# sanje2v/DualSuperResLearningForSemSeg

Hardware: AMD Instinct MI355X
Metric: stage-3 train images/sec at 256x512->512x1024 (higher is better)
Workload: dtype f32; 1 GPU; DSRL stage 3 (ResNet-101 OS16 + ASPP + SSSR/SISR decoders + FA loss), full train step, random-init weights, 256x512 input -> 512x1024 logits; global_batch=8, per_gpu_batch=8, parallelism=dp1, optimizer=SGD m0.9 wd5e-4 lr0.006

## Files before the change

dualsuperreslearningforsemseg_amd/_lib.py:

```python
import ctypes as C
import os

import torch

_HERE = os.path.dirname(os.path.abspath(__file__))
LIB_PATH = os.path.join(_HERE, 'libdsrl_hip.so')

fp = C.c_void_p
i32 = C.c_int
i64 = C.c_int64
u64 = C.c_uint64
u32 = C.c_uint32
f32 = C.c_float
sz = C.c_size_t
stream_t = C.c_void_p

_conv_shape = [i32] * 10


class WgradProblem(C.Structure):
    _fields_ = [('x', C.c_void_p), ('dy', C.c_void_p), ('dw', C.c_void_p)] + [(n, C.c_int32) for n in
                ('ldx', 'lddy', 'N', 'H', 'W', 'C', 'K', 'R', 'S', 'stride', 'pad', 'dil')] + [('x_amax', C.c_void_p), ('dy_amax', C.c_void_p)]


PROTOTYPES = {
    'dsrl_version': (i32, []),
    'dsrl_last_error': (C.c_char_p, []),
    'dsrl_device_check': (i32, [C.POINTER(i32)]),
    'dsrl_conv2d_fwd_workspace_bytes': (sz, _conv_shape),
    'dsrl_conv2d_fwd': (i32, [fp, i32, fp, fp, fp, i32] + _conv_shape + [fp, sz, stream_t]),
    'dsrl_conv2d_fwd_stats_parts': (i32, _conv_shape),
    'dsrl_conv2d_fwd_stats': (i32, [fp, i32, fp, fp, fp, i32] + _conv_shape + [fp, sz, fp, i32, stream_t]),
    'dsrl_conv2d_dgrad_workspace_bytes': (sz, _conv_shape),
    'dsrl_conv2d_transposed_filter_floats': (sz, [i32] * 4),
    'dsrl_conv2d_transpose_filter': (i32, [fp, fp, i32, i32, i32, i32, stream_t]),
    'dsrl_conv2d_transpose_filters_batched': (i32, [fp, i32, i64, stream_t]),
    'dsrl_conv2d_filters_amax_segment_floats': (i32, []),
    'dsrl_conv2d_filters_amax_batched': (i32, [fp, i64, stream_t]),
    'dsrl_conv2d_dgrad': (i32, [fp, i32, fp, fp, fp, i32] + _conv_shape + [fp, sz, stream_t]),
    'dsrl_conv2d_dgrad_stats_parts': (i32, _conv_shape),
    'dsrl_conv2d_dgrad_bnstats': (i32, [fp, i32, fp, fp, fp, i32] + _conv_shape + [fp, sz, fp, i32, fp, i32, fp, fp, i32, fp, i32, i32, stream_t]),
    'dsrl_conv2d_dgrad_accumulate': (i32, [fp, i32, fp, fp, fp, i32] + _conv_shape + [fp, sz, stream_t]),
    'dsrl_conv2d_wgrad_workspace_bytes': (sz, _conv_shape),
    'dsrl_conv2d_wgrad': (i32, [fp, i32, fp, i32, fp] + _conv_shape + [fp, sz, stream_t]),
    'dsrl_conv2d_wgrad_group_table_bytes': (sz, [i32]),
    'dsrl_conv2d_wgrad_group_workspace_bytes': (sz, [fp, i32]),
    'dsrl_conv2d_wgrad_group_plan': (i32, [fp, i32, fp, sz, fp, fp, sz]),
    'dsrl_conv2d_wgrad_group_launch': (i32, [fp, fp, stream_t]),
    'dsrl_amax': (i32, [fp, i32, i64, i32, fp, stream_t]),
    'dsrl_conv2d_fwd_amax': (i32, [fp, i32, fp, fp, fp, fp, fp, fp, i32] + _conv_shape + [fp, sz, fp, i32, stream_t]),
    'dsrl_conv2d_dgrad_amax': (i32, [fp, i32, fp, fp, fp, fp, fp, fp, i32] + _conv_shape + [fp, sz, fp, i32, fp, i32, fp, fp, i32, fp, i32, i32, stream_t]),
    'dsrl_conv2d_split_filters_batched': (i32, [fp, i32, i64, stream_t]),
    'dsrl_planes_lo_offset': (sz, [i64]),
    'dsrl_planes_bytes': (sz, [i64, i32]),
    'dsrl_split_planes': (i32, [fp, i32, i64, i32, fp, fp, i32, stream_t]),
    'dsrl_conv2d_filter_planes_batched': (i32, [fp, i32, i64, stream_t]),
    'dsrl_conv2d_fwd_planes': (i32, [fp, i32, fp, fp, fp, fp, fp, fp, fp, fp, i32] + _conv_shape + [fp, sz, fp, i32, stream_t]),
    'dsrl_conv2d_dgrad_planes': (i32, [fp, i32, fp, fp, fp, fp, fp, fp, fp, fp, i32] + _conv_shape + [fp, sz, fp, i32, fp, i32, fp, fp, i32, fp, i32, i32, stream_t]),
    'dsrl_conv2d_dgrad_planes_drop': (i32, [fp, i32, fp, fp, fp, fp, fp, fp, fp, fp, i32] + _conv_shape + [fp, sz, fp, i32, fp, i32, fp, fp, i32, f32, fp, i32, i32, stream_t]),
    'dsrl_conv2d_wgrad_amax': (i32, [fp, i32, fp, fp, i32, fp, fp] + _conv_shape + [fp, sz, stream_t]),
    'dsrl_conv_precision': (i32, [i32]),
    'dsrl_conv2d_inbounds_macs': (i64, _conv_shape),
    'dsrl_conv2d_rowfold_fwd_workspace_bytes': (sz, [i32] * 9),
    'dsrl_conv2d_rowfold_fwd': (i32, [fp, i32, fp, fp, fp, i32] + [i32] * 9 + [i64, fp, sz, stream_t]),
# ... 230 lines not shown
```

dualsuperreslearningforsemseg_amd/csrc/conv_common.h:

```cpp
#pragma once
#include "common.h"

namespace dsrl {

using f32x16 = __attribute__((ext_vector_type(16))) float;
using bf16x8 = __attribute__((ext_vector_type(8))) __bf16;
using bf16x4 = __attribute__((ext_vector_type(4))) __bf16;
using f16x8 = __attribute__((ext_vector_type(8))) _Float16;
using f16x4 = __attribute__((ext_vector_type(4))) _Float16;

template <bool F16> struct Plane;
template <> struct Plane<false> {
    using v4 = bf16x4; using v8 = bf16x8;
    static __device__ __forceinline__ v4 cvt(const float* r) { return v4{(__bf16)r[0], (__bf16)r[1], (__bf16)r[2], (__bf16)r[3]}; }
    static __device__ __forceinline__ void residual(float* r, v4 t) {
#pragma unroll
        for (int e = 0; e < 4; ++e) r[e] -= (float)t[e];
    }
    static __device__ __forceinline__ f32x16 mfma(v8 a, v8 b, f32x16 c) { return __builtin_amdgcn_mfma_f32_32x32x16_bf16(a, b, c, 0, 0, 0); }
};
__device__ __forceinline__ float f16_resid_lo(unsigned t, float r) { float d; asm("v_fma_mix_f32 %0, %1, -1.0, %2 op_sel:[0,0,0] op_sel_hi:[1,0,0]" : "=v"(d) : "v"(t), "v"(r)); return d; }
__device__ __forceinline__ float f16_resid_hi(unsigned t, float r) { float d; asm("v_fma_mix_f32 %0, %1, -1.0, %2 op_sel:[1,0,0] op_sel_hi:[1,0,0]" : "=v"(d) : "v"(t), "v"(r)); return d; }
template <> struct Plane<true> {
    using v4 = f16x4; using v8 = f16x8;
// ... 19 lines not shown
    return s == 255u ? n : q;
}

struct ConvArgs {
    const float* x; const float* w; const float* bias; float* y;
    int ldx, ldy;
    int N, H, W, C;
    int K;
    int R, S, Ho, Wo;
    int stride, pad, dil;
    int M;
    int cchunks;
    int splits;
    long long slab;
    unsigned x_bytes, w_bytes, y_bytes;
    int mtiles, ntiles, xcd_remap;
    int kg;
    int accumulate;
    float* stats;
    const float* bn_x; const float* bn_y; const float* bn_mean; const float* bn_invstd; float* bstats;
    int bn_ldx, bn_ldy, bn_relu;
    float bn_gscale;
    int bn_fast;
    int par, Hh, Wh, pbm;
    const unsigned* amax_a; const unsigned* amax_b;
    int w_split;
    unsigned mHW, sHW, mW, sW, mNT, sNT;
    unsigned a_lo, b_lo;
    int planes;
    float* coop_slab; unsigned* tickets;
};
constexpr int kCoopMaxTiles = (kAmaxShardStride - 1) * kAmaxShards;
__host__ __device__ inline int coop_ticket_word(int t) { return kAmaxShardStride * (t / (kAmaxShardStride - 1)) + 1 + t % (kAmaxShardStride - 1); }
__device__ __forceinline__ int dgrad_pix(const ConvArgs& a, int m) {
    const int t = m / a.pbm, p2 = a.par * a.par, c = t % p2, j = (t / p2) * a.pbm + (m - t * a.pbm);
    const int hw = a.Hh * a.Wh, n = j / hw, r = j - n * hw, hh = r / a.Wh, wh = r - hh * a.Wh;
    const int ph = c / a.par, pw = c - ph * a.par;
    return (n * a.Ho + hh * a.par + ph) * a.Wo + wh * a.par + pw;
}

__device__ __forceinline__ unsigned bn_mask_word(const ConvArgs& a, int k, long long px) {
    return reinterpret_cast<const unsigned*>(a.bn_y)[(long long)(k >> 5) * a.bn_ldy + px];
}
__device__ __forceinline__ float4 bn_mask4(unsigned w) { return make_float4((w & 1u) ? 1.f : 0.f, (w & 2u) ? 1.f : 0.f, (w & 4u) ? 1.f : 0.f, (w & 8u) ? 1.f : 0.f); }

__device__ inline int xcd_contiguous(int bid, int n) {
    const int q = n / kNumXCD, r = n % kNumXCD, xcd = bid % kNumXCD, local = bid / kNumXCD;
    return (xcd < r ? xcd * (q + 1) : r * (q + 1) + (xcd - r) * q) + local;
}

using u32x4 = __attribute__((ext_vector_type(4))) unsigned int;
constexpr unsigned kOOB = 0x80000000u;
__device__ inline float4 buf_load4(__amdgpu_buffer_rsrc_t r, unsigned off) {
    const u32x4 v = __builtin_amdgcn_raw_buffer_load_b128(r, (int)off, 0, 0);
    return make_float4(__uint_as_float(v.x), __uint_as_float(v.y), __uint_as_float(v.z), __uint_as_float(v.w));
}

struct WgradArgs {
    const float* x; const float* dy; float* dw;
    int ldx, lddy;
    int N, H, W, C, K, R, S, Ho, Wo, stride, pad, dil;
    long long P;
    unsigned x_bytes, dy_bytes;
    int ctiles;
    int psplits;
    long long slab;
    int taps[64]; int ntaps;
    int xcd_remap;
    int kctiles;
    unsigned mHW, sHW, mW, sW;
    int kg;
    int nblocks;
    float* dw_final;
    int rblocks;
    const unsigned* amax_dy; const unsigned* amax_x;
    int no_ident;
};

bool wgrad3_eligible(int N, int H, int W, int C, int K, int R, int S, int stride, int pad, int dil, int npl, bool f16);
// ... 13 lines not shown
```

dualsuperreslearningforsemseg_amd/csrc/conv_igemm.hip:

```cpp
#include "common.h"
#include "conv_common.h"
#include <algorithm>
#include <atomic>
#include <stdlib.h>
#include <string.h>
#include <mutex>
#include <vector>

namespace dsrl {

static std::atomic<int> g_conv_precision{-1};
constexpr int BK = 32;
constexpr int LDS_LD = 36;

template <int MR, int NR, int WGM, int WGN, bool DGRAD, int MINW = 2, bool = false>
__global__ __launch_bounds__(256, MINW) void conv_igemm_f32_kernel(const ConvArgs a) {
    constexpr int BM = 32 * MR * WGM, BN = 32 * NR * WGN;
    constexpr int A_IT = BM / 32, B_IT = BN / 32;
    extern __shared__ __attribute__((aligned(16))) float smem[];

    const int tid = threadIdx.x;
    const int lane = tid & 63;
    const int wave = __builtin_amdgcn_readfirstlane(tid >> 6);
    const int wm = wave / WGN, wn = wave % WGN;
// ... 1099 lines not shown
    unsigned* scratch = (unsigned*)((char*)ws + align_up(ws_used, 64));
    if (int e = launch_zero_fill(scratch, kAmaxScratch, st)) return e;
    if (am.a == nullptr) { if (int e = launch_amax(a, lda, Pa, Ca, scratch, st)) return e; am.a = scratch; }
    if (am.b == nullptr) { if (int e = launch_amax(b, ldb, Pb, Cb, scratch + kAmaxWords, st)) return e; am.b = scratch + kAmaxWords; }
    return DSRL_OK;
}

static void make_magic(int d, unsigned& m, unsigned& sh) {
    if (d <= 1) { m = 0; sh = 255u; return; }
    int l = 0;
    while ((1ll << l) < d) ++l;
    const unsigned long long k = 31 + l;
    m = (unsigned)((((unsigned long long)1 << k) + (unsigned long long)d - 1) / (unsigned long long)d);
    sh = (unsigned)(l - 1);
}
template <bool DGRAD>
static int launch_igemm(const ConvArgs& a_in, TileCfg cfg, hipStream_t st) {
    int bm, bn; cfg_dims(cfg, bm, bn);
    ConvArgs a = a_in;
    a.mtiles = (int)ceil_div(a.M, bm); a.ntiles = (int)ceil_div(a.K, bn);
    make_magic(a.Ho * a.Wo, a.mHW, a.sHW); make_magic(a.Wo, a.mW, a.sW); make_magic(a.ntiles, a.mNT, a.sNT);
    a.xcd_remap = knob("DSRL_XCD_REMAP", 1);
    if (a.bn_fast && !(DGRAD && conv_f16() && (size_t)bm * bn * 4 <= 128 * 1024)) a.bn_fast = 0;
    if (a.planes) return launch_planes_igemm(a, (int)cfg, DGRAD, st);
    dim3 grid((unsigned)(a.mtiles * a.ntiles), 1u, (unsigned)a.splits);
    const int npl = conv_planes(DGRAD ? PASS_DGRAD : PASS_FWD);
    const bool f16 = conv_f16();
    const long long nblocks = (long long)grid.x * grid.y * grid.z;
    if (f16 && (a.amax_a == nullptr || a.amax_b == nullptr)) { set_error("conv_igemm_split_kernel<f16x3>: operand magnitudes missing"); return DSRL_E_BADARG; }
    const bool s1 = DGRAD && a.stride == 1 && a.par == 0;
    if (npl) {
        const int kg = a.kg > 1 ? a.kg : 1;
        const size_t stages = (size_t)2 * (bm + bn) * npl * (f16 ? 64 : 32);
        if (kg > 1) {
            if (cfg == T128x128) {
                if (!sk_supported((int)cfg, kg, npl, f16, a.w_split != 0)) { set_error("conv_igemm_split_kernel: 128x128 tiles with two K groups exist for the fp16 arithmetics only"); return DSRL_E_UNSUPPORTED; }
                return launch_sk_igemm(a, DGRAD, s1, npl, st);
            }
            grid = dim3((unsigned)(a.mtiles * a.ntiles), 1u, (unsigned)std::max(1, a.splits));
            const size_t lds = std::max(stages * kg, (size_t)kg * (bm / 32) * (bn / 32) / 4 * 16384 + 8192);
#define DSRL_LAUNCH_KG(a_, b_, c_, d_, NPL_, KG_, F16_, S1_)                                                                          \
            {                                                                                                                          \
                static const hipError_t attr = hipFuncSetAttribute((const void*)conv_igemm_split_kernel<a_, b_, c_, d_, DGRAD, NPL_, KG_, F16_, S1_>, \
                                                                   hipFuncAttributeMaxDynamicSharedMemorySize, 128 * 1024);            \
                (void)attr;                                                                                                            \
                hipLaunchKernelGGL((conv_igemm_split_kernel<a_, b_, c_, d_, DGRAD, NPL_, KG_, F16_, S1_>), grid, dim3(256 * KG_), lds, st, a); \
            }
#define DSRL_KG_BY_ARITH(a_, b_, c_, d_, KG_) { if (f16 && npl == 1 && a.w_split) DSRL_LAUNCH_KG(a_, b_, c_, d_, 1, KG_, 2, false) else if (f16 && npl == 1) DSRL_LAUNCH_KG(a_, b_, c_, d_, 1, KG_, 1, false) else if (f16 && a.w_split && s1) DSRL_LAUNCH_KG(a_, b_, c_, d_, 2, KG_, 2, DGRAD) else if (f16 && a.w_split) DSRL_LAUNCH_KG(a_, b_, c_, d_, 2, KG_, 2, false) else if (f16) DSRL_LAUNCH_KG(a_, b_, c_, d_, 2, KG_, 1, false) else if (npl == 2) DSRL_LAUNCH_KG(a_, b_, c_, d_, 2, KG_, 0, false) else DSRL_LAUNCH_KG(a_, b_, c_, d_, 3, KG_, 0, false) }
            if (cfg == T64x64) {
                if (kg == 4) DSRL_KG_BY_ARITH(1, 1, 2, 2, 4) else DSRL_KG_BY_ARITH(1, 1, 2, 2, 2)
            } else if (cfg == T128x64) {
                DSRL_KG_BY_ARITH(2, 1, 2, 2, 2)
            } else {
                DSRL_KG_BY_ARITH(1, 2, 2, 2, 2)
            }
#undef DSRL_KG_BY_ARITH
#undef DSRL_LAUNCH_KG
            return launch_status("conv_igemm_split_kernel<K groups>");
        }
        const size_t lds2 = std::max(stages, a.bn_fast ? (size_t)bm * bn * 4 : (size_t)0);
        if (cfg == T256x128 || cfg == T256x256) {
#define DSRL_LAUNCH_BIG(a_, b_, c_, d_)                                                                                                   \
            {                                                                                                                              \
                if (f16 && npl == 1 && a.w_split) {                                                                                        \
                    static const hipError_t at_ = hipFuncSetAttribute((const void*)conv_igemm_split_kernel<a_, b_, c_, d_, DGRAD, 1, 1, 2, false>, hipFuncAttributeMaxDynamicSharedMemorySize, 128 * 1024); (void)at_; \
                    hipLaunchKernelGGL((conv_igemm_split_kernel<a_, b_, c_, d_, DGRAD, 1, 1, 2, false>), grid, dim3(512), lds2, st, a);      \
                } else if (f16 && npl == 1) {                                                                                              \
                    static const hipError_t at_ = hipFuncSetAttribute((const void*)conv_igemm_split_kernel<a_, b_, c_, d_, DGRAD, 1, 1, 1>, hipFuncAttributeMaxDynamicSharedMemorySize, 128 * 1024); (void)at_; \
                    hipLaunchKernelGGL((conv_igemm_split_kernel<a_, b_, c_, d_, DGRAD, 1, 1, 1>), grid, dim3(512), lds2, st, a);             \
                } else if (f16 && a.w_split && s1) {                                                                                       \
                    static const hipError_t at_ = hipFuncSetAttribute((const void*)conv_igemm_split_kernel<a_, b_, c_, d_, DGRAD, 2, 1, 2, DGRAD>, hipFuncAttributeMaxDynamicSharedMemorySize, 128 * 1024); (void)at_; \
                    hipLaunchKernelGGL((conv_igemm_split_kernel<a_, b_, c_, d_, DGRAD, 2, 1, 2, DGRAD>), grid, dim3(512), lds2, st, a);      \
                } else if (f16 && a.w_split) {                                                                                             \
                    static const hipError_t at_ = hipFuncSetAttribute((const void*)conv_igemm_split_kernel<a_, b_, c_, d_, DGRAD, 2, 1, 2>, hipFuncAttributeMaxDynamicSharedMemorySize, 128 * 1024); (void)at_; \
                    hipLaunchKernelGGL((conv_igemm_split_kernel<a_, b_, c_, d_, DGRAD, 2, 1, 2>), grid, dim3(512), lds2, st, a);             \
                } else if (f16) {                                                                                                          \
                    static const hipError_t at_ = hipFuncSetAttribute((const void*)conv_igemm_split_kernel<a_, b_, c_, d_, DGRAD, 2, 1, 1>, hipFuncAttributeMaxDynamicSharedMemorySize, 128 * 1024); (void)at_; \
                    hipLaunchKernelGGL((conv_igemm_split_kernel<a_, b_, c_, d_, DGRAD, 2, 1, 1>), grid, dim3(512), lds2, st, a);             \
                } else {                                                                                                                   \
                    set_error("conv_igemm_split_kernel: the 8-wave tiles exist for the f16x3 arithmetic only"); return DSRL_E_UNSUPPORTED;   \
                }                                                                                                                          \
            }
            if (cfg == T256x128) DSRL_LAUNCH_BIG(2, 2, 4, 2)
// ... 350 lines not shown
        a.y = slabs; a.ldy = C; a.bias = nullptr;
        if (int e = launch_igemm<true>(a, p.cfg, st)) return e;
        const long long total = (long long)p.M * C;
        hipLaunchKernelGGL(splitk_reduce_kernel, dim3((unsigned)std::min<long long>(ceil_div(total, 256), 4096)), dim3(256), 0, st,
                           (const float*)slabs, p.splits, a.slab, p.M, C, (const float*)nullptr, dx, lddx, accumulate);
        return launch_status("splitk_reduce_kernel");
    }
    if (p.splits > 1) {
        a.coop_slab = slabs; a.tickets = const_cast<unsigned*>(a.amax_a);
        a.y_bytes = (unsigned)span_bytes(p.M, lddx, C);
    }
    a.y = dx; a.ldy = lddx; a.bias = nullptr; a.accumulate = accumulate;
    if (stride > 1 && conv_planes(PASS_DGRAD) && H % stride == 0 && W % stride == 0 && (W / stride) % 32 == 0 && knob("DSRL_DGRAD_PARITY", 1)) {
        int bm, bn_; cfg_dims(p.cfg, bm, bn_);
        const long long Mc = (long long)N * (H / stride) * (W / stride);
        if (Mc % bm == 0) { a.par = stride; a.Hh = H / stride; a.Wh = W / stride; a.pbm = bm; }
    }
    if (bn) {
        a.bn_x = bn->x; a.bn_y = bn->y; a.bn_mean = bn->mean; a.bn_invstd = bn->invstd; a.bstats = bn->stats; a.bn_ldx = bn->ldx; a.bn_ldy = bn->ldy; a.bn_relu = bn->relu;
        a.bn_gscale = bn->gscale;
        const bool y4 = bn->relu != 1 || (bn->ldy % 4 == 0 && ((uintptr_t)bn->y % 16) == 0);
        a.bn_fast = a.par == 0 && C % 4 == 0 && bn->ldx % 4 == 0 && y4 && ((uintptr_t)bn->x % 16) == 0 &&
                    ((uintptr_t)bn->mean % 16) == 0 && ((uintptr_t)bn->invstd % 16) == 0 && ((uintptr_t)bn->stats % 16) == 0;
    }
    return launch_igemm<true>(a, p.cfg, st);
}

extern "C" int dsrl_conv2d_dgrad(const float* dy, int lddy, const float* w, const float* wt_in, float* dx, int lddx,
                                 int N, int H, int W, int C, int K, int R, int S, int stride, int pad, int dil,
                                 void* ws, size_t ws_bytes, dsrl_stream_t stream) {
    return dgrad_impl(dy, lddy, w, wt_in, dx, lddx, N, H, W, C, K, R, S, stride, pad, dil, ws, ws_bytes, stream, 0);
}
extern "C" int dsrl_conv2d_dgrad_stats_parts(int N, int H, int W, int C, int K, int R, int S, int stride, int pad, int dil) {
    const int Ho = out_size(H, R, stride, pad, dil), Wo = out_size(W, S, stride, pad, dil);
    if (Ho <= 0 || Wo <= 0) return 0;
    const int npl = conv_planes(PASS_DGRAD);
    return fwd_stats_parts(plan_dgrad(N, Ho, Wo, pad4(K), C, R, S, H, W, npl, stride), npl, true);
}
extern "C" int dsrl_conv2d_dgrad_bnstats(const float* dy, int lddy, const float* w, const float* wt_in, float* dx, int lddx,
                                         int N, int H, int W, int C, int K, int R, int S, int stride, int pad, int dil,
                                         void* ws, size_t ws_bytes, const float* bn_x, int bn_ldx, const float* bn_y, int bn_ldy,
                                         const float* bn_mean, const float* bn_invstd, int bn_relu, float* bstats, int stats_parts, int accumulate,
                                         dsrl_stream_t stream) {
    DSRL_REQUIRE(bn_x && bn_mean && bn_invstd && bstats && bn_ldx >= C && bn_y_ok(bn_y, bn_ldy, bn_relu, N, H, W, C), DSRL_E_BADARG, "conv2d_dgrad_bnstats: bad BatchNorm arguments");
    DSRL_REQUIRE(dsrl_conv2d_dgrad_stats_parts(N, H, W, C, K, R, S, stride, pad, dil) == stats_parts && stats_parts > 0, DSRL_E_BADARG,
                 "conv2d_dgrad_bnstats: this launch writes %d row blocks of partials, the caller expects %d",
                 dsrl_conv2d_dgrad_stats_parts(N, H, W, C, K, R, S, stride, pad, dil), stats_parts);
    DgradBn bn{bn_x, bn_y, bn_mean, bn_invstd, bstats, bn_ldx, bn_ldy, bn_relu};
    return dgrad_impl(dy, lddy, w, wt_in, dx, lddx, N, H, W, C, K, R, S, stride, pad, dil, ws, ws_bytes, stream, accumulate ? 1 : 0, &bn);
}
extern "C" int dsrl_conv2d_dgrad_accumulate(const float* dy, int lddy, const float* w, const float* wt_in, float* dx, int lddx,
                                            int N, int H, int W, int C, int K, int R, int S, int stride, int pad, int dil,
                                            void* ws, size_t ws_bytes, dsrl_stream_t stream) {
    return dgrad_impl(dy, lddy, w, wt_in, dx, lddx, N, H, W, C, K, R, S, stride, pad, dil, ws, ws_bytes, stream, 1);
// ... 569 lines not shown
```

dualsuperreslearningforsemseg_amd/csrc/conv_planes.hip:

```cpp
#include "common.h"
#include "conv_common.h"
#include "lds_dma.h"
#include <algorithm>

namespace dsrl {

template <int NPL> struct PlaneMfma;
template <> struct PlaneMfma<2> {
    template <int MR, int NR>
    static __device__ __forceinline__ void run(f32x16 (&acc)[MR][NR], const f16x8 (&fa)[MR][2], const f16x8 (&fb)[NR][2]) {
#pragma unroll
        for (int sum = 1; sum >= 0; --sum)
#pragma unroll
            for (int pa = 0; pa <= sum; ++pa)
#pragma unroll
                for (int i = 0; i < MR; ++i)
#pragma unroll
                    for (int j = 0; j < NR; ++j)
                        acc[i][j] = __builtin_amdgcn_mfma_f32_32x32x16_f16(fa[i][pa], fb[j][sum - pa], acc[i][j], 0, 0, 0);
    }
};
template <> struct PlaneMfma<1> {
    template <int MR, int NR>
    static __device__ __forceinline__ void run(f32x16 (&acc)[MR][NR], const f16x8 (&fa)[MR][1], const f16x8 (&fb)[NR][1]) {
// ... 249 lines not shown
            for (int jj = 0; jj < NR; ++jj)
#pragma unroll
                for (int e = 0; e < 16; ++e) acc[i][jj][e] = __builtin_ldexpf(acc[i][jj][e], sh);
    }
    float mine[KG > 1 ? MR : 1][KG > 1 ? NR : 1][KG > 1 ? EPG : 1];
    if constexpr (KG > 1) {
#pragma unroll
        for (int g = 0; g < KG; ++g)
            if (grp == g) {
#pragma unroll
                for (int i = 0; i < MR; ++i)
#pragma unroll
                    for (int j = 0; j < NR; ++j)
#pragma unroll
                        for (int k = 0; k < EPG; ++k) mine[i][j][k] = acc[i][j][g * EPG + k];
            }
    }
    auto share = [&](int i, int j, int e) -> float { if constexpr (KG > 1) return mine[i][j][e]; else return acc[i][j][e]; };
    auto share_add = [&](int i, int j, int e, float v) { if constexpr (KG > 1) mine[i][j][e] += v; else acc[i][j][e] += v; };
    const int rowg = 8 * ((grp * EPG) >> 2);
    float* yout = a.y + (a.splits > 1 ? (long long)z * a.slab : 0ll);
    const __amdgpu_buffer_rsrc_t yr = __builtin_amdgcn_make_buffer_rsrc((void*)yout, 0, (int)a.y_bytes, 0x00020000);
    const int col = lane & 31, rq = (lane >> 5) * 4 + rowg;
#pragma unroll
    for (int j = 0; j < NR; ++j) {
        const int k = n0 + (wn * NR + j) * 32 + col;
        const bool kok = k < a.K;
        const float bv = (a.bias != nullptr && kok) ? a.bias[k] : 0.f;
#pragma unroll
        for (int i = 0; i < MR; ++i) {
            const int mb32 = m0 + (wm * MR + i) * 32, mb = mb32 + rq;
            if (a.accumulate && a.splits == 1) {
                float old[EPG];
#pragma unroll
                for (int e = 0; e < EPG; ++e) {
                    const int m = mb + (e & 3) + 8 * (e >> 2);
                    const unsigned off = (kok && m < a.M) ? ((unsigned)m * (unsigned)a.ldy + (unsigned)k) * 4u : kOOB;
                    old[e] = __uint_as_float(__builtin_amdgcn_raw_buffer_load_b32(yr, (int)off, 0, 0));
                }
#pragma unroll
                for (int e = 0; e < EPG; ++e) share_add(i, j, e, old[e]);
            }
#pragma unroll
            for (int e = 0; e < EPG; ++e) {
                const int m = mb + (e & 3) + 8 * (e >> 2);
                const unsigned off = (kok && m < a.M) ? ((unsigned)m * (unsigned)a.ldy + (unsigned)k) * 4u : kOOB;
                __builtin_amdgcn_raw_buffer_store_b32(__float_as_uint(share(i, j, e) + bv), yr, (int)off, 0, 0);
            }
        }
    }
    bool bstats_done = false;
    if constexpr (DGRAD && KG == 1) {
        if (a.bstats != nullptr && (a.splits == 1) && a.bn_fast) {
            constexpr int TR = 32 * MR, TC = 32 * NR, CQ = TC / 4, RSTEP = 64 / CQ, NIT = TR / RSTEP, NB = NIT < 8 ? NIT : 8;
            float* wt = reinterpret_cast<float*>(smem) + (size_t)wave * TR * TC;
            __syncthreads();
#pragma unroll
            for (int i = 0; i < MR; ++i)
#pragma unroll
                for (int j = 0; j < NR; ++j)
#pragma unroll
                    for (int e = 0; e < 16; ++e)
                        wt[(i * 32 + (e & 3) + 8 * (e >> 2) + 4 * (lane >> 5)) * TC + j * 32 + (lane & 31)] = acc[i][j][e];
            const int c4 = lane % CQ, r0_ = lane / CQ;
            const int kk = n0 + wn * TC + 4 * c4;
            const bool kok4 = kk < a.K;
            const float4 mu4 = kok4 ? *reinterpret_cast<const float4*>(a.bn_mean + kk) : make_float4(0.f, 0.f, 0.f, 0.f);
            const float4 is4 = kok4 ? *reinterpret_cast<const float4*>(a.bn_invstd + kk) : make_float4(0.f, 0.f, 0.f, 0.f);
            float sg[4] = {0.f, 0.f, 0.f, 0.f}, sgx[4] = {0.f, 0.f, 0.f, 0.f};
            const int mrow0 = m0 + wm * TR;
#pragma unroll
            for (int b0 = 0; b0 < NIT; b0 += NB) {
                float4 xv[NB], yv[NB];
#pragma unroll
                for (int u = 0; u < NB; ++u) {
                    const int m = mrow0 + r0_ + RSTEP * (b0 + u);
// ... 246 lines not shown
                    for (int q = 0; q < 4; ++q) { r0[q] = __builtin_ldexpf(tile[g8 + q][row], sh); r1[q] = __builtin_ldexpf(tile[g8 + 4 + q][row], sh); }
                    const f16x4 t0 = Plane<true>::cvt(r0), t1 = Plane<true>::cvt(r1);
                    Plane<true>::residual(r0, t0); Plane<true>::residual(r1, t1);
                    const uint2 h0 = __builtin_bit_cast(uint2, t0), h1 = __builtin_bit_cast(uint2, t1);
                    const uint2 l0 = __builtin_bit_cast(uint2, Plane<true>::cvt(r0)), l1 = __builtin_bit_cast(uint2, Plane<true>::cvt(r1));
                    const long long off = (((long long)c * RS + tap) * K + k) * 2;
                    *reinterpret_cast<uint4*>(wtp + off) = make_uint4(h0.x, h0.y, h1.x, h1.y);
                    *reinterpret_cast<uint4*>(wtp + lo_off + off) = make_uint4(l0.x, l0.y, l1.x, l1.y);
                }
            }
        }
    }
}

#define DSRL_PLANES_LAUNCH_N(MR_, NR_, WGM_, WGN_, KG_, NPL_, R_)                                                                          \
    {                                                                                                                                       \
        constexpr int threads = 64 * WGM_ * WGN_ * KG_;                                                                                     \
        constexpr size_t slot = (size_t)(32 * MR_ * WGM_ + 32 * NR_ * WGN_) * NPL_ * 64;                                                   \
        constexpr size_t redb = KG_ > 1 ? (size_t)KG_ * MR_ * NR_ * 4 * (threads / KG_) * 16 + 8192 : 0;                                    \
        constexpr size_t tileb = (KG_ == 1 && DGRAD) ? (size_t)(32 * MR_ * WGM_) * (32 * NR_ * WGN_) * 4 : 0;       \
        constexpr size_t lds0 = slot * R_ * KG_ > redb ? slot * R_ * KG_ : redb;                                                            \
        constexpr size_t lds = (tileb > lds0 && tileb <= 160 * 1024) ? tileb : lds0;                                                        \
        static_assert(lds <= 160 * 1024, "LDS");                                                                                            \
        static const hipError_t attr = hipFuncSetAttribute((const void*)conv_planes_kernel<MR_, NR_, WGM_, WGN_, KG_, NPL_, DGRAD, R_>,      \
                                                           hipFuncAttributeMaxDynamicSharedMemorySize, (int)lds);                           \
        (void)attr;                                                                                                                         \
        hipLaunchKernelGGL((conv_planes_kernel<MR_, NR_, WGM_, WGN_, KG_, NPL_, DGRAD, R_>), grid, dim3(threads), lds, st, a);               \
        return launch_status("conv_planes_kernel");                                                                                         \
    }
#define DSRL_PLANES_LAUNCH2(MR_, NR_, WGM_, WGN_, KG_, R_, R1_) { if (a.planes == 1) DSRL_PLANES_LAUNCH_N(MR_, NR_, WGM_, WGN_, KG_, 1, R1_) else DSRL_PLANES_LAUNCH_N(MR_, NR_, WGM_, WGN_, KG_, 2, R_) }
#define DSRL_PLANES_LAUNCH(MR_, NR_, WGM_, WGN_, KG_, R_) DSRL_PLANES_LAUNCH2(MR_, NR_, WGM_, WGN_, KG_, R_, R_)

template <bool DGRAD>
static int launch_planes_t(const ConvArgs& a, int cfg, hipStream_t st) {
    if (a.kg > 1 && a.splits > 1) { set_error("conv_planes_kernel: no launch for %d K groups with %d split-K slabs", a.kg, a.splits); return DSRL_E_UNSUPPORTED; }
    const dim3 grid((unsigned)(a.mtiles * a.ntiles), 1u, (unsigned)(a.kg > 1 ? 1 : a.splits));
    const int kg = a.kg > 1 ? a.kg : 1;
    switch (cfg) {
        case 3:
            if (kg == 4) DSRL_PLANES_LAUNCH2(1, 1, 2, 2, 4, 2, 4)
            if (kg == 2) DSRL_PLANES_LAUNCH(1, 1, 2, 2, 2, 4)
            DSRL_PLANES_LAUNCH(1, 1, 2, 2, 1, 3)
        case 4:
            if (kg == 2) DSRL_PLANES_LAUNCH(2, 1, 2, 2, 2, 3)
            if (kg == 1) DSRL_PLANES_LAUNCH(2, 1, 2, 2, 1, 3)
            break;
// ... 67 lines not shown
```

dualsuperreslearningforsemseg_amd/csrc/conv_sk.hip:

```cpp
#include "common.h"
#include "conv_common.h"
#include "conv_split_kernel.h"
#include <algorithm>

namespace dsrl {

constexpr size_t kSkStages = (size_t)2 * (128 + 128) * 2 * 64 * 2;
constexpr size_t kSkReduce = (size_t)2 * 2 * 2 * 4 * 256 * 16 + 8192;
constexpr size_t kSkLds = kSkStages > kSkReduce ? kSkStages : kSkReduce;
static_assert(kSkLds <= 160 * 1024, "LDS");
size_t sk_lds_bytes() { return kSkLds; }

bool sk_supported(int cfg, int kg, int npl, bool f16, bool w_split) {
    (void)w_split;
    return cfg == 0 && (kg == 2 || kg == 1) && f16 && (npl == 1 || npl == 2);
}

template <bool DGRAD, int NPL, int ARITH, bool STR1, int KG>
static int launch_one_kg(const ConvArgs& a, hipStream_t st) {
    auto* k = conv_igemm_split_kernel<2, 2, 2, 2, DGRAD, NPL, KG, ARITH, STR1, true>;
    static const hipError_t attr = hipFuncSetAttribute((const void*)k, hipFuncAttributeMaxDynamicSharedMemorySize, (int)kSkLds);
    (void)attr;
    const dim3 grid((unsigned)(a.mtiles * a.ntiles), 1u, (unsigned)a.splits);
    const size_t lds = KG > 1 ? kSkLds : std::max((size_t)2 * (128 + 128) * NPL * 64, a.bn_fast ? (size_t)128 * 128 * 4 : (size_t)0);
    hipLaunchKernelGGL(k, grid, dim3(256 * KG), lds, st, a);
    return launch_status("conv_igemm_split_kernel<128x128, cooperative split-K>");
}
template <bool DGRAD, int NPL, int ARITH, bool STR1>
static int launch_one(const ConvArgs& a, hipStream_t st) {
    return a.kg > 1 ? launch_one_kg<DGRAD, NPL, ARITH, STR1, 2>(a, st) : launch_one_kg<DGRAD, NPL, ARITH, STR1, 1>(a, st);
}

int launch_sk_igemm(const ConvArgs& a, bool dgrad, bool str1, int npl, hipStream_t st) {
    if (a.splits > 1 && a.tickets != nullptr) {
        if (a.coop_slab == nullptr || a.mtiles * a.ntiles > kCoopMaxTiles) { set_error("cooperative split-K: no slab, or more than %d tiles", kCoopMaxTiles); return DSRL_E_BADARG; }
        if ((long long)a.splits * a.mtiles * a.ntiles * 128 * 128 * 4 >= (1ll << 31)) { set_error("cooperative split-K: partial tiles exceed the 2 GiB descriptor range"); return DSRL_E_UNSUPPORTED; }
    }
    if (npl == 2) {
        if (a.w_split) {
            if (dgrad) return str1 ? launch_one<true, 2, 2, true>(a, st) : launch_one<true, 2, 2, false>(a, st);
            return launch_one<false, 2, 2, false>(a, st);
        }
        return dgrad ? launch_one<true, 2, 1, false>(a, st) : launch_one<false, 2, 1, false>(a, st);
    }
    if (a.w_split) return dgrad ? launch_one<true, 1, 2, false>(a, st) : launch_one<false, 1, 2, false>(a, st);
    return dgrad ? launch_one<true, 1, 1, false>(a, st) : launch_one<false, 1, 1, false>(a, st);
}
// ... 3 lines not shown
```

dualsuperreslearningforsemseg_amd/csrc/conv_split_kernel.h:

```cpp
#pragma once
#include "common.h"
#include "conv_common.h"

namespace dsrl {

template <int MR, int NR, int WGM, int WGN, bool DGRAD, int NPL, int KG = 1, int ARITH = 0, bool STR1 = false, bool COOP = false>
__global__ __launch_bounds__(64 * WGM * WGN * KG, KG == 1 ? 2 : 1)
void conv_igemm_split_kernel(const ConvArgs a) {
    const int stride = STR1 ? 1 : a.stride, par = STR1 ? 0 : a.par;
    constexpr bool F16 = ARITH != 0, PREB = ARITH == 2;
    constexpr int NT = 64 * WGM * WGN, RP = NT / 4;
    static_assert(NT == 256 || (NT == 512 && KG == 1), "4 waves per K group, or one group of 8 waves");
    static_assert(!F16 || NPL <= 2, "f16x3 carries two fp16 terms per operand, f16x1 one");
    using PT = Plane<F16>;
    using pl4 = typename PT::v4; using pl8 = typename PT::v8;
    const unsigned am_a = F16 ? amax_fetch(a.amax_a) : 0u, am_b = F16 ? amax_fetch(a.amax_b) : 0u;
    int sh_a = 0, sh_b = 0;
    constexpr int BM = 32 * MR * WGM, BN = 32 * NR * WGN;
    constexpr int A_IT = (BM + RP - 1) / RP, B_IT = (BN + RP - 1) / RP;
    constexpr int NV = A_IT + B_IT;
    constexpr bool FS = F16;
    constexpr int ROWB = FS ? 64 : 32;
    constexpr int STAGE = (BM + BN) * NPL * ROWB;
    extern __shared__ __attribute__((aligned(16))) float smem[];
// ... 416 lines not shown
#pragma unroll
                    for (int i = 0; i < MR; ++i)
#pragma unroll
                        for (int j = 0; j < NR; ++j)
#pragma unroll
                            for (int k = 0; k < EPG; ++k) xch[((i * NR + j) * 16 + grp * EPG + k) * 256 + tid] = mine[i][j][k];
                    __syncthreads();
                    if (grp == 0) {
#pragma unroll
                        for (int i = 0; i < MR; ++i)
#pragma unroll
                            for (int j = 0; j < NR; ++j)
#pragma unroll
                                for (int e = 0; e < 16; ++e) acc[i][j][e] = xch[((i * NR + j) * 16 + e) * 256 + tid];
                    }
                }
            }
        }
    }
    const bool single = coop || a.splits == 1;
    float* yout = a.y + (!single ? (long long)z * a.slab : 0ll);
    const __amdgpu_buffer_rsrc_t yr = __builtin_amdgcn_make_buffer_rsrc((void*)yout, 0, (int)a.y_bytes, 0x00020000);
    const int col = lane & 31, rq = (lane >> 5) * 4 + rowg;
#pragma unroll
    for (int j = 0; j < NR; ++j) {
        const int k = n0 + (wn * NR + j) * 32 + col;
        const bool kok = k < a.K;
        const float bv = (a.bias != nullptr && kok) ? a.bias[k] : 0.f;
#pragma unroll
        for (int i = 0; i < MR; ++i) {
            const int mb32 = m0 + (wm * MR + i) * 32, mb = mb32 + rq;
            const int pix0 = (DGRAD && par) ? dgrad_pix(a, min(mb32, a.M - 1)) : mb32, pst = (DGRAD && par) ? par : 1;
            if (a.accumulate && single) {
                float old[EPG];
#pragma unroll
                for (int e = 0; e < EPG; ++e) {
                    const int m = mb + (e & 3) + 8 * (e >> 2);
                    const unsigned off = (kok && m < a.M) ? ((unsigned)(pix0 + (m - mb32) * pst) * (unsigned)a.ldy + (unsigned)k) * 4u : kOOB;
                    old[e] = __uint_as_float(__builtin_amdgcn_raw_buffer_load_b32(yr, (int)off, 0, 0));
                }
#pragma unroll
                for (int e = 0; e < EPG; ++e) share_add(i, j, e, old[e]);
            }
#pragma unroll
            for (int e = 0; e < EPG; ++e) {
                const int m = mb + (e & 3) + 8 * (e >> 2);
                const unsigned off = (kok && m < a.M) ? ((unsigned)(pix0 + (m - mb32) * pst) * (unsigned)a.ldy + (unsigned)k) * 4u : kOOB;
                __builtin_amdgcn_raw_buffer_store_b32(__float_as_uint(share(i, j, e) + bv), yr, (int)off, 0, 0);
            }
        }
    }
    bool bstats_done = false;
    if constexpr (DGRAD && KG == 1) {
        if (a.bstats != nullptr && single && a.bn_fast) {
            constexpr int TR = 32 * MR, TC = 32 * NR, CQ = TC / 4, RSTEP = 64 / CQ, NIT = TR / RSTEP, NB = NIT < 8 ? NIT : 8;
            float* wt = reinterpret_cast<float*>(smem) + (size_t)wave * TR * TC;
            __syncthreads();
#pragma unroll
            for (int i = 0; i < MR; ++i)
#pragma unroll
                for (int j = 0; j < NR; ++j)
#pragma unroll
                    for (int e = 0; e < 16; ++e)
                        wt[(i * 32 + (e & 3) + 8 * (e >> 2) + 4 * (lane >> 5)) * TC + j * 32 + (lane & 31)] = acc[i][j][e];
            const int c4 = lane % CQ, r0_ = lane / CQ;
            const int kk = n0 + wn * TC + 4 * c4;
            const bool kok4 = kk < a.K;
            const float4 mu4 = kok4 ? *reinterpret_cast<const float4*>(a.bn_mean + kk) : make_float4(0.f, 0.f, 0.f, 0.f);
            const float4 is4 = kok4 ? *reinterpret_cast<const float4*>(a.bn_invstd + kk) : make_float4(0.f, 0.f, 0.f, 0.f);
            float sg[4] = {0.f, 0.f, 0.f, 0.f}, sgx[4] = {0.f, 0.f, 0.f, 0.f};
            const int mrow0 = m0 + wm * TR;
#pragma unroll
            for (int b0 = 0; b0 < NIT; b0 += NB) {
                float4 xv[NB], yv[NB];
#pragma unroll
                for (int u = 0; u < NB; ++u) {
                    const int m = mrow0 + r0_ + RSTEP * (b0 + u);
// ... 157 lines not shown
```

include/dsrl_hip.h:

```cpp
#ifndef DSRL_HIP_H
#define DSRL_HIP_H

#include <stddef.h>
#include <stdint.h>

#ifdef __cplusplus
extern "C" {
#endif

#define DSRL_ABI_VERSION 1

#define DSRL_OK 0
#define DSRL_E_BADARG (-1)
#define DSRL_E_UNSUPPORTED (-2)
#define DSRL_E_WORKSPACE (-3)
#define DSRL_E_LAUNCH (-4)

typedef void* dsrl_stream_t;

int dsrl_version(void);
const char* dsrl_last_error(void);
int dsrl_device_check(int* cu_count);

size_t dsrl_conv2d_fwd_workspace_bytes(int N, int H, int W, int C, int K, int R, int S, int stride, int pad, int dil);
// ... 1 lines not shown
                    int N, int H, int W, int C, int K, int R, int S, int stride, int pad, int dil,
                    void* ws, size_t ws_bytes, dsrl_stream_t stream);
int dsrl_conv2d_fwd_stats_parts(int N, int H, int W, int C, int K, int R, int S, int stride, int pad, int dil);
int dsrl_conv2d_fwd_stats(const float* x, int ldx, const float* w, const float* bias , float* y, int ldy,
                          int N, int H, int W, int C, int K, int R, int S, int stride, int pad, int dil,
                          void* ws, size_t ws_bytes, float* stats, int stats_parts, dsrl_stream_t stream);
size_t dsrl_conv2d_transposed_filter_floats(int C, int K, int R, int S);
int dsrl_conv2d_transpose_filter(const float* w, float* wt, int C, int K, int R, int S, dsrl_stream_t stream);
int dsrl_conv2d_transpose_filters_batched(const int64_t* table, int n, int64_t total_tiles, dsrl_stream_t stream);
int dsrl_conv2d_filters_amax_segment_floats(void);
int dsrl_conv2d_filters_amax_batched(const int64_t* table, int64_t nseg, dsrl_stream_t stream);

int dsrl_conv2d_split_filters_batched(const int64_t* table, int n, int64_t total_tiles, dsrl_stream_t stream);
size_t dsrl_conv2d_dgrad_workspace_bytes(int N, int H, int W, int C, int K, int R, int S, int stride, int pad, int dil);
int dsrl_conv2d_dgrad(const float* dy, int lddy, const float* w, const float* wt , float* dx, int lddx,
                      int N, int H, int W, int C, int K, int R, int S, int stride, int pad, int dil,
                      void* ws, size_t ws_bytes, dsrl_stream_t stream);
int dsrl_conv2d_dgrad_stats_parts(int N, int H, int W, int C, int K, int R, int S, int stride, int pad, int dil);
int dsrl_conv2d_dgrad_bnstats(const float* dy, int lddy, const float* w, const float* wt , float* dx, int lddx,
                              int N, int H, int W, int C, int K, int R, int S, int stride, int pad, int dil,
                              void* ws, size_t ws_bytes, const float* bn_x, int bn_ldx, const float* bn_y , int bn_ldy,
                              const float* bn_mean, const float* bn_invstd, int bn_relu, float* bstats, int stats_parts,
                              int accumulate , dsrl_stream_t stream);
int dsrl_conv2d_dgrad_accumulate(const float* dy, int lddy, const float* w, const float* wt , float* dx, int lddx,
                                 int N, int H, int W, int C, int K, int R, int S, int stride, int pad, int dil,
                                 void* ws, size_t ws_bytes, dsrl_stream_t stream);
size_t dsrl_conv2d_wgrad_workspace_bytes(int N, int H, int W, int C, int K, int R, int S, int stride, int pad, int dil);
int dsrl_conv2d_wgrad(const float* x, int ldx, const float* dy, int lddy, float* dw,
                      int N, int H, int W, int C, int K, int R, int S, int stride, int pad, int dil,
                      void* ws, size_t ws_bytes, dsrl_stream_t stream);
typedef struct dsrl_wgrad_problem {
    const float* x; const float* dy; float* dw;
    int32_t ldx, lddy, N, H, W, C, K, R, S, stride, pad, dil;
    const uint32_t* x_amax; const uint32_t* dy_amax;
} dsrl_wgrad_problem;
size_t dsrl_conv2d_wgrad_group_table_bytes(int n);
size_t dsrl_conv2d_wgrad_group_workspace_bytes(const dsrl_wgrad_problem* problems, int n);
int dsrl_conv2d_wgrad_group_plan(const dsrl_wgrad_problem* problems, int n, void* host_table, size_t table_bytes, const void* dev_table,
                                 void* ws, size_t ws_bytes);
int dsrl_conv2d_wgrad_group_launch(const void* host_table, const void* dev_table, dsrl_stream_t stream);
#define DSRL_AMAX_WORDS 256
int dsrl_amax(const float* x, int ld, int64_t P, int C, uint32_t* amax, dsrl_stream_t stream);
int dsrl_conv2d_fwd_amax(const float* x, int ldx, const uint32_t* x_amax, const float* w, const uint32_t* w_amax, const void* w_split ,
                         const float* bias , float* y, int ldy, int N, int H, int W, int C, int K, int R, int S, int stride, int pad, int dil,
                         void* ws, size_t ws_bytes, float* stats , int stats_parts, dsrl_stream_t stream);
int dsrl_conv2d_dgrad_amax(const float* dy, int lddy, const uint32_t* dy_amax, const float* w, const float* wt , const uint32_t* w_amax,
// ... 437 lines not shown
```

Before: 503.2 images/s.

## Add row-major LDS-staged dgrad epilogue with coalesced accumulate and BN-stat fusion

Adds a RowEpilogue that parks the MFMA accumulator tile in LDS per wave. It then re-reads the tile row-wise so the dgrad output accumulate, bias add, store and BN backward statistics use 128-bit coalesced buffer loads and stores. The old destination values and BN inputs are prefetched before the LDS park to hide their latency. This targets the column-strided scalar epilogue of the accumulate and bn-stats dgrad paths in f16 mode. In exchange it uses more LDS and registers for the prefetched rows, and adds a guard that rejects builds with insufficient LDS.

```diff
diff --git a/dualsuperreslearningforsemseg_amd/_lib.py b/dualsuperreslearningforsemseg_amd/_lib.py
--- a/dualsuperreslearningforsemseg_amd/_lib.py
+++ b/dualsuperreslearningforsemseg_amd/_lib.py
@@ -40,6 +40,7 @@
     'dsrl_conv2d_dgrad': (i32, [fp, i32, fp, fp, fp, i32] + _conv_shape + [fp, sz, stream_t]),
     'dsrl_conv2d_dgrad_stats_parts': (i32, _conv_shape),
     'dsrl_conv2d_dgrad_bnstats': (i32, [fp, i32, fp, fp, fp, i32] + _conv_shape + [fp, sz, fp, i32, fp, i32, fp, fp, i32, fp, i32, i32, stream_t]),
+    'dsrl_conv2d_row_epilogue_supported': (i32, [i32] * 10 + [sz] + [i32] * 4),
     'dsrl_conv2d_dgrad_accumulate': (i32, [fp, i32, fp, fp, fp, i32] + _conv_shape + [fp, sz, stream_t]),
     'dsrl_conv2d_wgrad_workspace_bytes': (sz, _conv_shape),
     'dsrl_conv2d_wgrad': (i32, [fp, i32, fp, i32, fp] + _conv_shape + [fp, sz, stream_t]),
diff --git a/dualsuperreslearningforsemseg_amd/csrc/conv_common.h b/dualsuperreslearningforsemseg_amd/csrc/conv_common.h
--- a/dualsuperreslearningforsemseg_amd/csrc/conv_common.h
+++ b/dualsuperreslearningforsemseg_amd/csrc/conv_common.h
@@ -65,6 +65,8 @@
     int bn_ldx, bn_ldy, bn_relu;
     float bn_gscale;
     int bn_fast;
+    int row_epi;
+    unsigned bn_x_bytes, bn_y_bytes;
     int par, Hh, Wh, pbm;
     const unsigned* amax_a; const unsigned* amax_b;
     int w_split;
@@ -98,6 +100,109 @@
     const u32x4 v = __builtin_amdgcn_raw_buffer_load_b128(r, (int)off, 0, 0);
     return make_float4(__uint_as_float(v.x), __uint_as_float(v.y), __uint_as_float(v.z), __uint_as_float(v.w));
 }
+
+template <int MR, int NR>
+struct RowEpilogue {
+    static constexpr int TR = 32 * MR, TC = 32 * NR, CQ = TC / 4, RSTEP = 64 / CQ, NIT = TR / RSTEP, NB = NIT < 8 ? NIT : 8;
+    int c4, r0, kk, mrow0;
+    bool kok4;
+    u32x4 old[NIT];
+    u32x4 xv[NB], yv[NB];
+    unsigned mw[NB];
+    float4 mu4, is4;
+
+    __device__ __forceinline__ void fetch_bn(const ConvArgs& a, __amdgpu_buffer_rsrc_t bx, __amdgpu_buffer_rsrc_t by, int b0) {
+#pragma unroll
+        for (int u = 0; u < NB; ++u) {
+            const int m = mrow0 + r0 + RSTEP * (b0 + u);
+            const bool ok = kok4 && m < a.M && a.bstats != nullptr;
+            xv[u] = __builtin_amdgcn_raw_buffer_load_b128(bx, (int)(ok ? ((unsigned)m * (unsigned)a.bn_ldx + (unsigned)kk) * 4u : kOOB), 0, 0);
+            yv[u] = __builtin_amdgcn_raw_buffer_load_b128(by, (int)((ok && a.bn_relu == 1) ? ((unsigned)m * (unsigned)a.bn_ldy + (unsigned)kk) * 4u : kOOB), 0, 0);
+            mw[u] = __builtin_amdgcn_raw_buffer_load_b32(by, (int)((ok && a.bn_relu == 2) ? ((unsigned)(kk >> 5) * (unsigned)a.bn_ldy + (unsigned)m) * 4u : kOOB), 0, 0);
+        }
+    }
+    __device__ __forceinline__ void fetch(const ConvArgs& a, __amdgpu_buffer_rsrc_t yr, __amdgpu_buffer_rsrc_t bx, __amdgpu_buffer_rsrc_t by, int lane, int mrow0_, int kcol0) {
+        c4 = lane % CQ; r0 = lane / CQ; mrow0 = mrow0_;
+        kk = kcol0 + 4 * c4;
+        kok4 = kk < a.K;
+#pragma unroll
+        for (int it = 0; it < NIT; ++it) {
+            const int m = mrow0 + r0 + RSTEP * it;
+            old[it] = __builtin_amdgcn_raw_buffer_load_b128(yr, (int)((kok4 && m < a.M && a.accumulate) ? ((unsigned)m * (unsigned)a.ldy + (unsigned)kk) * 4u : kOOB), 0, 0);
+        }
+        fetch_bn(a, bx, by, 0);
+        const bool st = kok4 && a.bstats != nullptr;
+        mu4 = st ? *reinterpret_cast<const float4*>(a.bn_mean + kk) : make_float4(0.f, 0.f, 0.f, 0.f);
+        is4 = st ? *reinterpret_cast<const float4*>(a.bn_invstd + kk) : make_float4(0.f, 0.f, 0.f, 0.f);
+    }
+    __device__ __forceinline__ void park(float* wt, const f32x16 (&acc)[MR][NR], int lane) const {
+#pragma unroll
+        for (int i = 0; i < MR; ++i)
+#pragma unroll
+            for (int j = 0; j < NR; ++j)
+#pragma unroll
+                for (int e = 0; e < 16; ++e)
+                    wt[(i * 32 + (e & 3) + 8 * (e >> 2) + 4 * (lane >> 5)) * TC + j * 32 + (lane & 31)] = acc[i][j][e];
+    }
+    __device__ __forceinline__ void pass(const ConvArgs& a, __amdgpu_buffer_rsrc_t yr, __amdgpu_buffer_rsrc_t bx, __amdgpu_buffer_rsrc_t by, const float* wt, int lane,
+                                         int part, int nparts) {
+        float bv[4];
+#pragma unroll
+        for (int e = 0; e < 4; ++e) bv[e] = (a.bias != nullptr && kok4) ? a.bias[kk + e] : 0.f;
+        const bool sums = a.bstats != nullptr;
+        float sg[4] = {0.f, 0.f, 0.f, 0.f}, sgx[4] = {0.f, 0.f, 0.f, 0.f};
+#pragma unroll
+        for (int b0 = 0; b0 < NIT; b0 += NB) {
+            if (b0 > 0) fetch_bn(a, bx, by, b0);
+#pragma unroll
+            for (int u = 0; u < NB; ++u) {
+                const int row = r0 + RSTEP * (b0 + u), m = mrow0 + row;
+                const bool ok = kok4 && m < a.M;
+                float4 gv = *reinterpret_cast<const float4*>(wt + row * TC + 4 * c4);
+                if (a.accumulate) {
+                    const u32x4 o = old[b0 + u];
+                    gv.x += __uint_as_float(o.x); gv.y += __uint_as_float(o.y); gv.z += __uint_as_float(o.z); gv.w += __uint_as_float(o.w);
+                }
+                const u32x4 q = {__float_as_uint(gv.x + bv[0]), __float_as_uint(gv.y + bv[1]), __float_as_uint(gv.z + bv[2]), __float_as_uint(gv.w + bv[3])};
+                __builtin_amdgcn_raw_buffer_store_b128(q, yr, (int)(ok ? ((unsigned)m * (unsigned)a.ldy + (unsigned)kk) * 4u : kOOB), 0, 0);
+                if (sums && ok) {
+                    float4 y4 = make_float4(1.f, 1.f, 1.f, 1.f);
+                    if (a.bn_relu == 2) y4 = bn_mask4(mw[u] >> (kk & 31));
+                    else if (a.bn_relu) y4 = make_float4(__uint_as_float(yv[u].x), __uint_as_float(yv[u].y), __uint_as_float(yv[u].z), __uint_as_float(yv[u].w));
+                    const float4 x4 = make_float4(__uint_as_float(xv[u].x), __uint_as_float(xv[u].y), __uint_as_float(xv[u].z), __uint_as_float(xv[u].w));
+                    const float gs = a.bn_gscale;
+                    const float g0 = (a.bn_relu && !(y4.x > 0.f)) ? 0.f : gv.x * gs, g1 = (a.bn_relu && !(y4.y > 0.f)) ? 0.f : gv.y * gs;
+                    const float g2 = (a.bn_relu && !(y4.z > 0.f)) ? 0.f : gv.z * gs, g3 = (a.bn_relu && !(y4.w > 0.f)) ? 0.f : gv.w * gs;
+                    sg[0] += g0; sgx[0] += g0 * ((x4.x - mu4.x) * is4.x);
+                    sg[1] += g1; sgx[1] += g1 * ((x4.y - mu4.y) * is4.y);
+                    sg[2] += g2; sgx[2] += g2 * ((x4.z - mu4.z) * is4.z);
+                    sg[3] += g3; sgx[3] += g3 * ((x4.w - mu4.w) * is4.w);
+                }
+            }
+        }
+        if (!sums) return;
+#pragma unroll
+        for (int sft = CQ; sft < 64; sft <<= 1)
+#pragma unroll
+            for (int q = 0; q < 4; ++q) { sg[q] += __shfl_xor(sg[q], sft); sgx[q] += __shfl_xor(sgx[q], sft); }
+        if (lane < CQ && kok4) {
+            float* o = a.bstats + (long long)part * a.K + kk;
+            *reinterpret_cast<float4*>(o) = make_float4(sg[0], sg[1], sg[2], sg[3]);
+            *reinterpret_cast<float4*>(o + (long long)nparts * a.K) = make_float4(sgx[0], sgx[1], sgx[2], sgx[3]);
+        }
+    }
+};
+
+inline bool row_epilogue_ok(const ConvArgs& a, bool dgrad, bool f16, int bm, int bn) {
+    if (!dgrad || !f16 || a.kg > 1 || a.stride != 1 || a.par != 0) return false;
+    if (a.splits > 1 && a.tickets == nullptr) return false;
+    if (a.K % 4 != 0 || a.ldy % 4 != 0 || ((uintptr_t)a.y % 16) != 0 || (size_t)bm * bn * 4 > 128 * 1024) return false;
+    if (a.bstats != nullptr && !(a.bn_fast && a.bn_x_bytes != 0 && (a.bn_relu == 0 || a.bn_y_bytes != 0))) return false;
+    if (!a.accumulate && a.bstats == nullptr) return false;
+    if (a.accumulate && a.stats != nullptr) return false;
+    return knob("DSRL_ROW_EPILOGUE", 1) != 0;
+}
+inline size_t epilogue_tile_bytes(const ConvArgs& a, int bm, int bn) { return (a.kg <= 1 && (a.bn_fast || a.row_epi)) ? (size_t)bm * bn * 4 : (size_t)0; }
 
 struct WgradArgs {
     const float* x; const float* dy; float* dw;
diff --git a/dualsuperreslearningforsemseg_amd/csrc/conv_igemm.hip b/dualsuperreslearningforsemseg_amd/csrc/conv_igemm.hip
--- a/dualsuperreslearningforsemseg_amd/csrc/conv_igemm.hip
+++ b/dualsuperreslearningforsemseg_amd/csrc/conv_igemm.hip
@@ -1145,6 +1145,7 @@
     make_magic(a.Ho * a.Wo, a.mHW, a.sHW); make_magic(a.Wo, a.mW, a.sW); make_magic(a.ntiles, a.mNT, a.sNT);
     a.xcd_remap = knob("DSRL_XCD_REMAP", 1);
     if (a.bn_fast && !(DGRAD && conv_f16() && (size_t)bm * bn * 4 <= 128 * 1024)) a.bn_fast = 0;
+    a.row_epi = row_epilogue_ok(a, DGRAD, conv_f16(), bm, bn) ? 1 : 0;
     if (a.planes) return launch_planes_igemm(a, (int)cfg, DGRAD, st);
     dim3 grid((unsigned)(a.mtiles * a.ntiles), 1u, (unsigned)a.splits);
     const int npl = conv_planes(DGRAD ? PASS_DGRAD : PASS_FWD);
@@ -1181,7 +1182,7 @@
 #undef DSRL_LAUNCH_KG
             return launch_status("conv_igemm_split_kernel<K groups>");
         }
-        const size_t lds2 = std::max(stages, a.bn_fast ? (size_t)bm * bn * 4 : (size_t)0);
+        const size_t lds2 = std::max(stages, epilogue_tile_bytes(a, bm, bn));
         if (cfg == T256x128 || cfg == T256x256) {
 #define DSRL_LAUNCH_BIG(a_, b_, c_, d_)                                                                                                   \
             {                                                                                                                              \
@@ -1578,6 +1579,10 @@
         const bool y4 = bn->relu != 1 || (bn->ldy % 4 == 0 && ((uintptr_t)bn->y % 16) == 0);
         a.bn_fast = a.par == 0 && C % 4 == 0 && bn->ldx % 4 == 0 && y4 && ((uintptr_t)bn->x % 16) == 0 &&
                     ((uintptr_t)bn->mean % 16) == 0 && ((uintptr_t)bn->invstd % 16) == 0 && ((uintptr_t)bn->stats % 16) == 0;
+        const long long bxb = span_bytes(p.M, bn->ldx, C);
+        const long long byb = bn->relu == 2 ? span_bytes(C / 32, bn->ldy, (int)std::min<long long>(p.M, bn->ldy)) : (bn->relu == 1 ? span_bytes(p.M, bn->ldy, C) : 0);
+        a.bn_x_bytes = bxb < (1ll << 31) ? (unsigned)bxb : 0u;
+        a.bn_y_bytes = byb < (1ll << 31) ? (unsigned)byb : 0u;
     }
     return launch_igemm<true>(a, p.cfg, st);
 }
@@ -1586,6 +1591,17 @@
                                  int N, int H, int W, int C, int K, int R, int S, int stride, int pad, int dil,
                                  void* ws, size_t ws_bytes, dsrl_stream_t stream) {
     return dgrad_impl(dy, lddy, w, wt_in, dx, lddx, N, H, W, C, K, R, S, stride, pad, dil, ws, ws_bytes, stream, 0);
+}
+extern "C" int dsrl_conv2d_row_epilogue_supported(int dgrad, int bm, int bn, int kg, int stride, int parity, int splits, int coop, int channels, int ldy,
+                                                  size_t y_addr, int accumulate, int bn_sums, int bn_fast, int fwd_stats) {
+    static unsigned word;
+    ConvArgs a{};
+    a.kg = kg; a.stride = stride; a.par = parity ? stride : 0; a.splits = splits > 1 ? splits : 1;
+    a.tickets = (a.splits > 1 && coop) ? &word : nullptr;
+    a.K = channels; a.ldy = ldy; a.y = (float*)y_addr; a.accumulate = accumulate ? 1 : 0;
+    a.bstats = bn_sums ? (float*)&word : nullptr; a.bn_fast = (bn_sums && bn_fast) ? 1 : 0; a.bn_x_bytes = a.bn_fast ? 4u : 0u; a.bn_relu = 0;
+    a.stats = fwd_stats ? (float*)&word : nullptr;
+    return row_epilogue_ok(a, dgrad != 0, conv_f16(), bm, bn) ? 1 : 0;
 }
 extern "C" int dsrl_conv2d_dgrad_stats_parts(int N, int H, int W, int C, int K, int R, int S, int stride, int pad, int dil) {
     const int Ho = out_size(H, R, stride, pad, dil), Wo = out_size(W, S, stride, pad, dil);
diff --git a/dualsuperreslearningforsemseg_amd/csrc/conv_planes.hip b/dualsuperreslearningforsemseg_amd/csrc/conv_planes.hip
--- a/dualsuperreslearningforsemseg_amd/csrc/conv_planes.hip
+++ b/dualsuperreslearningforsemseg_amd/csrc/conv_planes.hip
@@ -295,6 +295,22 @@
     float* yout = a.y + (a.splits > 1 ? (long long)z * a.slab : 0ll);
     const __amdgpu_buffer_rsrc_t yr = __builtin_amdgcn_make_buffer_rsrc((void*)yout, 0, (int)a.y_bytes, 0x00020000);
     const int col = lane & 31, rq = (lane >> 5) * 4 + rowg;
+    bool row_done = false;
+    if constexpr (DGRAD && KG == 1 && BM * BN * 4 <= 128 * 1024) {
+        if (a.row_epi && a.splits == 1) {
+            using RE = RowEpilogue<MR, NR>;
+            RE re;
+            const __amdgpu_buffer_rsrc_t bxr = __builtin_amdgcn_make_buffer_rsrc((void*)a.bn_x, 0, (int)a.bn_x_bytes, 0x00020000);
+            const __amdgpu_buffer_rsrc_t byr = __builtin_amdgcn_make_buffer_rsrc((void*)a.bn_y, 0, (int)a.bn_y_bytes, 0x00020000);
+            re.fetch(a, yr, bxr, byr, lane, m0 + wm * RE::TR, n0 + wn * RE::TC);
+            float* wt = reinterpret_cast<float*>(smem) + (size_t)wave * RE::TR * RE::TC;
+            __syncthreads();
+            re.park(wt, acc, lane);
+            re.pass(a, yr, bxr, byr, wt, lane, tile_m * WGM + wm, a.mtiles * WGM);
+            row_done = true;
+        }
+    }
+    if (!row_done)
 #pragma unroll
     for (int j = 0; j < NR; ++j) {
         const int k = n0 + (wn * NR + j) * 32 + col;
@@ -322,9 +338,9 @@
             }
         }
     }
-    bool bstats_done = false;
+    bool bstats_done = row_done;
     if constexpr (DGRAD && KG == 1) {
-        if (a.bstats != nullptr && (a.splits == 1) && a.bn_fast) {
+        if (a.bstats != nullptr && (a.splits == 1) && a.bn_fast && !row_done) {
             constexpr int TR = 32 * MR, TC = 32 * NR, CQ = TC / 4, RSTEP = 64 / CQ, NIT = TR / RSTEP, NB = NIT < 8 ? NIT : 8;
             float* wt = reinterpret_cast<float*>(smem) + (size_t)wave * TR * TC;
             __syncthreads();
@@ -617,6 +633,10 @@
         constexpr size_t lds0 = slot * R_ * KG_ > redb ? slot * R_ * KG_ : redb;                                                            \
         constexpr size_t lds = (tileb > lds0 && tileb <= 160 * 1024) ? tileb : lds0;                                                        \
         static_assert(lds <= 160 * 1024, "LDS");                                                                                            \
+        if (epilogue_tile_bytes(a, 32 * MR_ * WGM_, 32 * NR_ * WGN_) > lds) {       \
+            set_error("conv_planes_kernel: the epilogue parks %zu bytes, the build has %zu of LDS", epilogue_tile_bytes(a, 32 * MR_ * WGM_, 32 * NR_ * WGN_), lds); \
+            return DSRL_E_UNSUPPORTED;                                                                                                      \
+        }                                                                                                                                   \
         static const hipError_t attr = hipFuncSetAttribute((const void*)conv_planes_kernel<MR_, NR_, WGM_, WGN_, KG_, NPL_, DGRAD, R_>,      \
                                                            hipFuncAttributeMaxDynamicSharedMemorySize, (int)lds);                           \
         (void)attr;                                                                                                                         \
diff --git a/dualsuperreslearningforsemseg_amd/csrc/conv_sk.hip b/dualsuperreslearningforsemseg_amd/csrc/conv_sk.hip
--- a/dualsuperreslearningforsemseg_amd/csrc/conv_sk.hip
+++ b/dualsuperreslearningforsemseg_amd/csrc/conv_sk.hip
@@ -22,7 +22,7 @@
     static const hipError_t attr = hipFuncSetAttribute((const void*)k, hipFuncAttributeMaxDynamicSharedMemorySize, (int)kSkLds);
     (void)attr;
     const dim3 grid((unsigned)(a.mtiles * a.ntiles), 1u, (unsigned)a.splits);
-    const size_t lds = KG > 1 ? kSkLds : std::max((size_t)2 * (128 + 128) * NPL * 64, a.bn_fast ? (size_t)128 * 128 * 4 : (size_t)0);
+    const size_t lds = KG > 1 ? kSkLds : std::max((size_t)2 * (128 + 128) * NPL * 64, epilogue_tile_bytes(a, 128, 128));
     hipLaunchKernelGGL(k, grid, dim3(256 * KG), lds, st, a);
     return launch_status("conv_igemm_split_kernel<128x128, cooperative split-K>");
 }
diff --git a/dualsuperreslearningforsemseg_amd/csrc/conv_split_kernel.h b/dualsuperreslearningforsemseg_amd/csrc/conv_split_kernel.h
--- a/dualsuperreslearningforsemseg_amd/csrc/conv_split_kernel.h
+++ b/dualsuperreslearningforsemseg_amd/csrc/conv_split_kernel.h
@@ -462,6 +462,22 @@
     float* yout = a.y + (!single ? (long long)z * a.slab : 0ll);
     const __amdgpu_buffer_rsrc_t yr = __builtin_amdgcn_make_buffer_rsrc((void*)yout, 0, (int)a.y_bytes, 0x00020000);
     const int col = lane & 31, rq = (lane >> 5) * 4 + rowg;
+    bool row_done = false;
+    if constexpr (DGRAD && KG == 1 && BM * BN * 4 <= 128 * 1024) {
+        if (a.row_epi && single) {
+            using RE = RowEpilogue<MR, NR>;
+            RE re;
+            const __amdgpu_buffer_rsrc_t bxr = __builtin_amdgcn_make_buffer_rsrc((void*)a.bn_x, 0, (int)a.bn_x_bytes, 0x00020000);
+            const __amdgpu_buffer_rsrc_t byr = __builtin_amdgcn_make_buffer_rsrc((void*)a.bn_y, 0, (int)a.bn_y_bytes, 0x00020000);
+            re.fetch(a, yr, bxr, byr, lane, m0 + wm * RE::TR, n0 + wn * RE::TC);
+            float* wt = reinterpret_cast<float*>(smem) + (size_t)wave * RE::TR * RE::TC;
+            __syncthreads();
+            re.park(wt, acc, lane);
+            re.pass(a, yr, bxr, byr, wt, lane, tile_m * WGM + wm, a.mtiles * WGM);
+            row_done = true;
+        }
+    }
+    if (!row_done)
 #pragma unroll
     for (int j = 0; j < NR; ++j) {
         const int k = n0 + (wn * NR + j) * 32 + col;
@@ -490,9 +506,9 @@
             }
         }
     }
-    bool bstats_done = false;
+    bool bstats_done = row_done;
     if constexpr (DGRAD && KG == 1) {
-        if (a.bstats != nullptr && single && a.bn_fast) {
+        if (a.bstats != nullptr && single && a.bn_fast && !row_done) {
             constexpr int TR = 32 * MR, TC = 32 * NR, CQ = TC / 4, RSTEP = 64 / CQ, NIT = TR / RSTEP, NB = NIT < 8 ? NIT : 8;
             float* wt = reinterpret_cast<float*>(smem) + (size_t)wave * TR * TC;
             __syncthreads();
diff --git a/include/dsrl_hip.h b/include/dsrl_hip.h
--- a/include/dsrl_hip.h
+++ b/include/dsrl_hip.h
@@ -47,6 +47,8 @@
                               void* ws, size_t ws_bytes, const float* bn_x, int bn_ldx, const float* bn_y , int bn_ldy,
                               const float* bn_mean, const float* bn_invstd, int bn_relu, float* bstats, int stats_parts,
                               int accumulate , dsrl_stream_t stream);
+int dsrl_conv2d_row_epilogue_supported(int dgrad, int bm, int bn, int kg, int stride, int parity, int splits, int coop, int channels, int ldy,
+                                       size_t y_addr, int accumulate, int bn_sums, int bn_fast, int fwd_stats);
 int dsrl_conv2d_dgrad_accumulate(const float* dy, int lddy, const float* w, const float* wt , float* dx, int lddx,
                                  int N, int H, int W, int C, int K, int R, int S, int stride, int pad, int dil,
                                  void* ws, size_t ws_bytes, dsrl_stream_t stream);
```

After: 508.3 images/s, median of 6. 1.01x the previous value.
